# D-Robotics/hobot_stereonet

Measured on AMD Instinct MI355X. Metric: stereo pairs/s at 1280x720 D=192 (ms/frame alongside), higher is better.
Workload: dtype f16 (refinement-tower MFMA operands fp16 — 3x3 weights rounded per kernel so that every kernel's tap sum survives —, LeakyReLU applied after the fp16 rounding; low-resolution branch on 22-bit hi/lo split fp16 operands, 3 fp16 MFMAs per product in every 32-channel layer — profiles/r04_lowres_ablation

## Files before the change

hobot_stereonet_amd/csrc/sn_stream_block.hpp:

```cpp
#pragma once

#ifdef SN_STREAM_TIMING
#define SN_STAMP(k)                                                                                   \
  do {                                                                                                \
    if (blockIdx.x == 17 && q >= 8 && q < 24) {                                                       \
      const unsigned long long t_ = __builtin_readcyclecounter();                                     \
      if (lane == 0) reinterpret_cast<unsigned long long*>(dump + 64)[(wave * 16 + q - 8) * 8 + (k)] = t_; \
    }                                                                                                 \
  } while (0)
#define SN_STAMP_WG(k)                                                                                          \
  do {                                                                                                          \
    if (threadIdx.x == 0) {                                                                                     \
      unsigned long long* d_ = reinterpret_cast<unsigned long long*>(dump + 64) + 1152 + 4 * blockIdx.x + (k);  \
      d_[0] = __builtin_readcyclecounter();                                                                     \
      d_[2] = wall_clock64();                                                                                   \
    }                                                                                                           \
  } while (0)
#else
#define SN_STAMP(k) do { } while (0)
#define SN_STAMP_WG(k) do { } while (0)
#endif

namespace sn {

// ... 9 lines not shown
  static constexpr int LAG = HEAD_ ? 3 : 2;
  static constexpr int PROWS = 2 * R + 2;
  static constexpr int PRING_BYTES = HEAD_ ? PROWS * 9 * TW * 4 : 0;
  static constexpr int WIN_BYTES = HEAD_ ? NWR_ * 2 * 64 * 4 : 0;
  static constexpr int XW = TW + 2 * DIL;
  static constexpr int CSEG = TW / 32;
  static constexpr int SPW = R * CSEG / NWR;
  static constexpr int XROW = 4 * XW, TROW = 4 * TW;
  static constexpr int XGROUP = R * XROW;
  static constexpr int NINST = (XGROUP + 63) / 64;
  static constexpr int KW = (NINST + NWR - 1) / NWR;
  static constexpr int XGP = NINST * 64;
  static constexpr int TGP = R * TROW;
  static constexpr int XRING = NXS * XGP;
  static constexpr int TRING = NTS * TGP + 64;
  static constexpr int LDS_BYTES = (XRING + TRING) * 16 + 2 * 2 * 16 * 4 + PRING_BYTES + WIN_BYTES;
  static constexpr int ROWS_ABOVE = (R + HS) * DIL, ROWS_BELOW = (R + 2 + HS) * DIL - 1;
  static_assert(!HEAD_ || (DIL_ == 1 && R_ == 4 && TW_ == 64 && NWR_ == 4), "the tail form is written for the dilation-1 strip shape");
  static_assert(SPW == 1 || SPW == 2, "segments per wave");
  static_assert(CSEG % SPW == 0, "a wave's segments lie in one row");
  static_assert(PF == 2, "prefetch distance the counted waits are written for");
  static_assert(R == 4 || R == 2, "rows per step");
  static_assert(LDS_BYTES <= 160 * 1024, "one workgroup per CU");
};

struct StreamSched {
  int nstrips;
  int hsub;
  int total_rows;
  int rows_per_wg;
};

template <int R, int HS = 0>
struct StreamIter {
  int f, f_end, hsub;
  int sp, v0, v1, n, j, live;
  __device__ __forceinline__ void next_unit() {
    if (f >= f_end) { live = 0; return; }
    sp = f / hsub;
    v0 = f - sp * hsub;
    int L = hsub - v0;
    if (L > f_end - f) L = f_end - f;
    v1 = v0 + L;
    n = (L + 2 + 2 * HS + R - 1) / R;
    j = 0;
    f += L;
    live = 1;
  }
  __device__ __forceinline__ void step(int q, int lag, int f0, int f1, int hsub_) {
    if (q < lag) { live = 0; return; }
    if (q == lag) { f = f0; f_end = f1; hsub = hsub_; next_unit(); return; }
    if (live && ++j > n) next_unit();
  }
};

__device__ __forceinline__ unsigned lrelu_pack2(float a, float b) { return act_pack2_f16(a, b, (_Float16)kSlope); }

template <int HI>
__device__ __forceinline__ float res_add(unsigned r, float acc) {
  float d;
  if (HI) asm("v_fma_mix_f32 %0, %1, 1.0, %2 op_sel:[1,0,0] op_sel_hi:[1,0,0]" : "=v"(d) : "v"(r), "v"(acc));
  else asm("v_fma_mix_f32 %0, %1, 1.0, %2 op_sel_hi:[1,0,0]" : "=v"(d) : "v"(r), "v"(acc));
  return d;
}

__device__ __forceinline__ unsigned lds_addr(const void* p) {
  return (unsigned)(size_t)(const __attribute__((address_space(3))) void*)p;
}

// ... 33 lines not shown
  }
  __builtin_amdgcn_sched_group_barrier(0x008, AHEAD, 0);
}

__device__ __forceinline__ void glds16(unsigned lds_dst, unsigned voff, const void* base) {
  unsigned keep;
  asm volatile(
      "s_mov_b32 %0, m0\n\t"
      "s_mov_b32 m0, %1\n\t"
      "s_nop 0\n\t"
      "global_load_lds_dwordx4 %2, %3\n\t"
      "s_mov_b32 m0, %0"
      : "=&s"(keep)
      : "s"(lds_dst), "v"(voff), "s"(base)
      : "memory");
}

__device__ __forceinline__ void glds4(unsigned lds_dst, unsigned voff, const void* base) {
  unsigned keep;
  asm volatile(
      "s_mov_b32 %0, m0\n\t"
      "s_mov_b32 m0, %1\n\t"
      "s_nop 0\n\t"
      "global_load_lds_dword %2, %3\n\t"
      "s_mov_b32 m0, %0"
      : "=&s"(keep)
      : "s"(lds_dst), "v"(voff), "s"(base)
      : "memory");
}

// ... 3 lines not shown
                                                                const uint4* __restrict__ wfrag2, const float* __restrict__ bias2,
                                                                RefGeom g, StreamSched sc, uint4* __restrict__ dump, HeadArgs ha) {
  using T = StreamTile<DIL, TW, R, NXS, NWR, HEAD>;
  constexpr int HS = T::HS;
  extern __shared__ __attribute__((aligned(16))) uint4 lds[];
  uint4* const xring = lds;
  uint4* const tring = lds + T::XRING;
  float* const s_bias = reinterpret_cast<float*>(tring + T::TRING);
  float* const pring = s_bias + 64;
  float* const s_win = pring + T::PRING_BYTES / 4;
  const int tid = threadIdx.x, lane = tid & 63;
  const int wave = __builtin_amdgcn_readfirstlane(tid >> 6);
  const int j = lane & 31, gh = lane >> 5;
  const int role = wave / NWR, rw = wave % NWR;

  const int f0 = (int)blockIdx.x * sc.rows_per_wg;
  int f1 = f0 + sc.rows_per_wg;
  if (f1 > sc.total_rows) f1 = sc.total_rows;
  if (f0 >= f1) return;
  SN_STAMP_WG(0);
  int nss = T::LAG;
  for (int f = f0; f < f1;) {
    const int v0 = f % sc.hsub;
    int L = sc.hsub - v0;
    if (L > f1 - f) L = f1 - f;
    nss += (L + 2 + 2 * HS + R - 1) / R + 1;
    f += L;
  }
  auto decode_sp = [&](int sp, int& img, int& py, int& x0) {
    const int t = sp / sc.nstrips;
    x0 = (sp - t * sc.nstrips) * T::OW + T::X0OFF;
    img = t / DIL;
    py = t - img * DIL;
  };
  const unsigned plane_b = (unsigned)g.Hs * (unsigned)g.Ws * 16u;

  half8 wf[18];
  {
    const uint4* wsrc = role ? wfrag2 : wfrag1;
#pragma unroll
    for (int i = 0; i < 18; ++i) {
      const uint4 a = wsrc[i * 64 + lane];
      wf[i] = *reinterpret_cast<const half8*>(&a);
    }
    if (tid < 64) {
      const int c = tid >> 5, g2 = (tid >> 4) & 1, r = tid & 15;
      s_bias[tid] = (c ? bias2 : bias1)[(r & 3) + 8 * (r >> 2) + 4 * g2];
    }
#pragma unroll
// ... 12 lines not shown
    const int lane_w = cseg0 * 32 + j;
    constexpr int KWMAX = T::KW;
    const int kw = (T::NINST - rw + NWR - 1) / NWR;
    unsigned dma_voff[KWMAX];
#pragma unroll
    for (int k = 0; k < KWMAX; ++k) {
      const int i = rw + NWR * k;
      int s = i * 64 + lane;
      s = s < T::XGROUP ? s : T::XGROUP - 1;
      const int r = s / T::XROW;
      const int rem = s - r * T::XROW;
      const int blk = rem / T::XW;
      const int c = rem - blk * T::XW;
      dma_voff[k] = (unsigned)blk * plane_b + ((unsigned)(r * DIL) * (unsigned)g.Ws + (unsigned)c) * 16u;
    }
    long last_base = 0;
    auto dma_issue = [&](const StreamIter<R, HS>& it, int grp) {
      if (it.live) {
        int img, py, x0;
        decode_sp(it.sp, img, py, x0);
        const int row = (it.v0 - HS - R + R * it.j) * DIL + py;
        last_base = (((long)img * 4 * g.Hs + (row + kRefPad)) * (long)g.Ws + (x0 - 2 * DIL + kRefPad)) * 16;
      }
      const char* src = reinterpret_cast<const char*>(xin) + last_base;
      const unsigned dst = lds_addr(xring + grp * T::XGP);
#pragma unroll
      for (int k = 0; k < KWMAX; ++k)
        if (k < kw) glds16(dst + (unsigned)(rw + NWR * k) * 1024u, dma_voff[k], src);
    };
    auto wait_group = [&](auto extra) {
      constexpr int E = decltype(extra)::value;
      if (kw == KWMAX) wait_vmcnt<KWMAX + E>();
      else wait_vmcnt<KWMAX - 1 + E>();
    };
    StreamIter<R, HS> dm, c1, fin, fin2;
    dm.live = c1.live = fin.live = fin2.live = 0;
    int fin_img = 0, fin_x0 = 0, fin2_img = 0, fin2_x0 = 0;
    auto win_first_col = [&](int xs) {
      float sx = ((float)xs + 0.5f) * ha.ups.rs - 0.5f;
      sx = sx < 0.f ? 0.f : sx;
      return (int)sx;
    };
    int p4 = 0;
    unsigned long long moved = 0ull;
    unsigned bad = 0u;
    dm.step(0, 0, f0, f1, sc.hsub);
    dma_issue(dm, 0);
    dm.step(1, 0, f0, f1, sc.hsub);
    dma_issue(dm, 1);
    wait_group(std::integral_constant<int, 0>{});
    block_barrier();

    int c1_py = 0, c1_x0 = 0;
    int qx = 0, qt = 0;
    for (int q = 0; q < nss; ++q) {
      dm.step(q + 2, 0, f0, f1, sc.hsub);
      c1.step(q, 0, f0, f1, sc.hsub);
      const int do1 = c1.live && c1.j >= 1;
      const int gx0 = qx, gx1 = qx >= 1 ? qx - 1 : qx - 1 + NXS;
      const int gxp = qx + 2 >= NXS ? qx + 2 - NXS : qx + 2;
      SN_STAMP(0);
      if constexpr (HEAD) {
        fin.step(q, 3, f0, f1, sc.hsub);
        if (fin.live && fin.j >= 1) {
          if (fin.j == 1) {
            int py;
            decode_sp(fin.sp, fin_img, py, fin_x0);
          }
          const int o = fin.v0 - 4 + R * (fin.j - 1) + rowW;
          if (o >= fin.v0 && o < fin.v1 && o < ha.H) {
            const int pb = p4 + 8 >= T::PROWS ? p4 + 8 - T::PROWS : p4 + 8;
            float acc = ha.bias;
#pragma unroll
            for (int ky = 0; ky < 3; ++ky) {
              int pr = pb + rowW - 2 + ky;
              pr = pr < 0 ? pr + T::PROWS : (pr >= T::PROWS ? pr - T::PROWS : pr);
              const float* prow = pring + pr * (9 * TW) + lane - 1;
#pragma unroll
              for (int kx = 0; kx < 3; ++kx) acc += prow[(ky * 3 + kx) * TW + kx];
            }
            const int X = fin_x0 + lane;
            float sy = ((float)o + 0.5f) * ha.ups.rs - 0.5f;
            float sx = ((float)X + 0.5f) * ha.ups.rs - 0.5f;
            sy = sy < 0.f ? 0.f : sy;
            sx = sx < 0.f ? 0.f : sx;
            const int y0 = (int)sy, x0 = (int)sx;
            const int x1 = x0 < ha.wl - 1 ? x0 + 1 : x0;
            const float ly = sy - (float)y0, lx = sx - (float)x0;
            const float hy = 1.0f - ly, hx = 1.0f - lx;
            const int cb = win_first_col(fin_x0);
            const float* w0 = s_win + rw * 128;
            const float v = hy * (hx * w0[x0 - cb] + lx * w0[x1 - cb]) + ly * (hx * w0[64 + x0 - cb] + lx * w0[64 + x1 - cb]);
            const float up = v * ha.ups.mul;
            float mv;
            unsigned nf;
            const float d = head_value(up, ha.dmax, acc, mv, nf);
            if (lane >= 1 && lane <= T::OW && X < ha.W) {
              moved += stat_fixed(mv);
              bad += nf;
              head_store(ha.out_disp, ha.out_raw, ((size_t)fin_img * ha.H + o) * ha.W + X, d, ha.inv_q);
            }
          }
        }
      }
      if constexpr (HEAD) {
        fin2.step(q, 2, f0, f1, sc.hsub);
        if (fin2.live && fin2.j >= 1) {
          if (fin2.j == 1) {
            int py;
            decode_sp(fin2.sp, fin2_img, py, fin2_x0);
          }
          const int o = fin2.v0 - 4 + R * (fin2.j - 1) + rowW;
          if (o >= fin2.v0 && o < fin2.v1 && o < ha.H) {
            float sy = ((float)o + 0.5f) * ha.ups.rs - 0.5f;
            sy = sy < 0.f ? 0.f : sy;
            const int y0 = (int)sy;
            const int y1 = y0 < ha.hl - 1 ? y0 + 1 : y0;
            int c = win_first_col(fin2_x0) + lane;
            c = c < ha.wl - 1 ? c : ha.wl - 1;
            const float* lowp = ha.disp_low + (size_t)fin2_img * ha.hl * ha.wl;
            const unsigned dst = lds_addr(s_win + rw * 128);
            asm volatile("s_waitcnt lgkmcnt(0)" ::: "memory");
            glds4(dst, (unsigned)c * 4u, lowp + (size_t)y0 * ha.wl);
            glds4(dst + 256u, (unsigned)c * 4u, lowp + (size_t)y1 * ha.wl);
          }
        }
      }
      dma_issue(dm, gxp);
      SN_STAMP(1);
      if (do1) {
        if (c1.j == 1) {
          int img;
          decode_sp(c1.sp, img, c1_py, c1_x0);
        }
        const uint4* xp[3];
#pragma unroll
        for (int ky = 0; ky < 3; ++ky) {
          const int rr = rowW - 2 + ky;
          xp[ky] = xring + (rr < 0 ? gx1 : gx0) * T::XGP + (rr & (R - 1)) * T::XROW + lane_x;
        }
        const f32x16 bv = *reinterpret_cast<const f32x16*>(s_bias + gh * 16);
        f32x16 acc[T::SPW];
        stream_conv36<DIL, T::XW, T::SPW>(xp, wf, bv, acc);
        SN_STAMP(2);
        const int trow = (c1.v0 - HS - 1 + R * (c1.j - 1) + rowW) * DIL + c1_py;
        const bool row_ok = trow >= 0 && trow < g.H;
        const int tc0 = c1_x0 - DIL;
        const bool interior = row_ok && tc0 >= 0 && tc0 + TW <= g.W;
        uint4* tw = tring + qt * T::TGP + rowW * T::TROW + lane_w;
        auto write_t = [&](auto is_interior) {
#pragma unroll
          for (int s = 0; s < T::SPW; ++s) {
            bool inside = true;
            if (!decltype(is_interior)::value) {
              const int c = tc0 + (cseg0 + s) * 32 + j;
              inside = row_ok && c >= 0 && c < g.W;
            }
            unsigned pk[4][2];
#pragma unroll
            for (int qd = 0; qd < 4; ++qd)
// ... 14 lines not shown
      wait_group(std::integral_constant<int, 0>{});
      asm volatile("s_waitcnt lgkmcnt(0)" ::: "memory");
      SN_STAMP(4);
      block_barrier();
      qx = qx + 1 == NXS ? 0 : qx + 1;
      qt = qt + 1 == T::NTS ? 0 : qt + 1;
      p4 = p4 + R >= T::PROWS ? p4 + R - T::PROWS : p4 + R;
    }
    if constexpr (HEAD) refine_stat_commit_fixed(ha.stat, moved, bad);
    SN_STAMP_WG(1);
  } else {
    const int lane_t = gh * T::TW + cseg0 * 32 + j;
    const int lane_y = 2 * DIL + cseg0 * 32 + j;
    block_barrier();

    StreamIter<R, HS> c2, ep;
    c2.live = ep.live = 0;
    half8 ah[2], al[2];
    uint2 rres[T::SPW][4];
    int p4 = 0;
    if constexpr (HEAD) {
#pragma unroll
      for (int kk = 0; kk < 2; ++kk)
#pragma unroll
        for (int e = 0; e < 8; ++e) {
          const float wv = j < 9 ? ha.w[(16 * kk + 8 * gh + e) * 9 + j] : 0.f;
          const _Float16 hi = (_Float16)wv;
          ah[kk][e] = hi;
          al[kk][e] = (_Float16)((wv - (float)hi) * kSplitScale);
        }
#pragma unroll
      for (int s = 0; s < T::SPW; ++s)
#pragma unroll
        for (int qd = 0; qd < 4; ++qd) rres[s][qd] = uint2{0u, 0u};
    }
    int ep_img = 0, ep_py = 0, ep_x0 = 0;
    const unsigned lane_o = (unsigned)(cseg0 * 32 + j) * 16u + (unsigned)(2 * gh) * plane_b;
    f32x16 acc[T::SPW];
#pragma unroll
    for (int s = 0; s < T::SPW; ++s)
#pragma unroll
      for (int r = 0; r < 16; ++r) acc[s][r] = 0.f;
    int qx = 0, qt = 0;
    for (int q = 0; q < nss; ++q) {
      c2.step(q, 1, f0, f1, sc.hsub);
      ep.step(q, 2, f0, f1, sc.hsub);
      const int do2 = c2.live && c2.j >= 1;
      const int doe = ep.live && ep.j >= 1;
      const int gx2 = qx >= 2 ? qx - 2 : qx - 2 + NXS, gx3 = qx >= 3 ? qx - 3 : qx - 3 + NXS;
      const int gt1 = qt >= 1 ? qt - 1 : qt - 1 + T::NTS, gt2 = qt >= 2 ? qt - 2 : qt - 2 + T::NTS;
      SN_STAMP(0);
      if (doe) {
        if (ep.j == 1) decode_sp(ep.sp, ep_img, ep_py, ep_x0);
        const int sub = ep.v0 - HS - 2 + R * (ep.j - 1) + rowW;
        const int row = sub * DIL + ep_py;
        if constexpr (HEAD) {
          const bool row_ok = row >= 0 && row < g.H;
          const bool interior = row_ok && ep_x0 >= 0 && ep_x0 + TW <= g.W;
          int prow = p4 + 2 + rowW;
          prow = prow >= T::PROWS ? prow - T::PROWS : prow;
#pragma unroll
          for (int s = 0; s < T::SPW; ++s) {
            const int col = ep_x0 + (cseg0 + s) * 32 + j;
            const bool ok = row_ok && col >= 0 && col < g.W;
            unsigned pk[4][2];
#pragma unroll
            for (int qd = 0; qd < 4; ++qd) {
              const half4 rv = *reinterpret_cast<const half4*>(&rres[s][qd]);
              const uint2 rw2 = *reinterpret_cast<const uint2*>(&rv);
// ... 16 lines not shown
#pragma unroll
            for (int kk = 0; kk < 2; ++kk) {
              const auto r0 = __builtin_amdgcn_permlane32_swap(pk[2 * kk][0], pk[2 * kk + 1][0], false, false);
              const auto r1 = __builtin_amdgcn_permlane32_swap(pk[2 * kk][1], pk[2 * kk + 1][1], false, false);
              const uint4 sl = uint4{r0[0], r1[0], r0[1], r1[1]};
              const half8 xh = *reinterpret_cast<const half8*>(&sl);
              a0 = __builtin_amdgcn_mfma_f32_32x32x16_f16(ah[kk], xh, a0, 0, 0, 0);
              a1 = __builtin_amdgcn_mfma_f32_32x32x16_f16(al[kk], xh, a1, 0, 0, 0);
            }
            float* dst = pring + prow * (9 * TW) + (cseg0 + s) * 32 + j;
#pragma unroll
            for (int r = 0; r < 4; ++r) dst[(4 * gh + r) * TW] = a0[r] + a1[r] * kSplitInv;
            if (gh == 0) dst[8 * TW] = a0[4] + a1[4] * kSplitInv;
          }
        } else
        if (sub >= ep.v0 && sub < ep.v1 && row < g.H) {
          const int rr = rowW - 2;
          const uint4* xrow = xring + (rr < 0 ? gx3 : gx2) * T::XGP + (rr & (R - 1)) * T::XROW + lane_y;
          const unsigned ob = (((unsigned)ep_img * 4u * (unsigned)g.Hs + (unsigned)(row + kRefPad)) * (unsigned)g.Ws +
                               (unsigned)(ep_x0 + kRefPad)) * 16u;
#pragma unroll
          for (int s = 0; s < T::SPW; ++s) {
            unsigned pk[4][2];
#pragma unroll
            for (int qd = 0; qd < 4; ++qd) {
              const half4 rv = *reinterpret_cast<const half4*>(reinterpret_cast<const char*>(xrow + qd * T::XW + s * 32) + gh * 8);
              const uint2 rw2 = *reinterpret_cast<const uint2*>(&rv);
              pk[qd][0] = lrelu_pack2(res_add<0>(rw2.x, acc[s][4 * qd]), res_add<1>(rw2.x, acc[s][4 * qd + 1]));
              pk[qd][1] = lrelu_pack2(res_add<0>(rw2.y, acc[s][4 * qd + 2]), res_add<1>(rw2.y, acc[s][4 * qd + 3]));
            }
            uint4 sl[2];
#pragma unroll
            for (int k = 0; k < 2; ++k) {
              const auto r0 = __builtin_amdgcn_permlane32_swap(pk[k][0], pk[k + 2][0], false, false);
              const auto r1 = __builtin_amdgcn_permlane32_swap(pk[k][1], pk[k + 2][1], false, false);
// ... 47 lines not shown
```

hobot_stereonet_amd/csrc/sn_stream_block_x3.hpp:

```cpp
#pragma once

namespace sn {

template <int DIL_, int TW_ = 64, int R_ = 2, int NXS_ = 5, int NWR_ = 2>
struct StreamTileX3 {
  static constexpr int DIL = DIL_, TW = TW_, R = R_, NXS = NXS_, NTS = 3, PF = NXS_ - 3;
  static constexpr int NWR = NWR_;
  static constexpr int OW = TW - 2 * DIL;
  static constexpr int XW = TW + 2 * DIL;
  static constexpr int CSEG = TW / 32;
  static constexpr int SPW = R * CSEG / NWR;
  static constexpr int XROW = 4 * XW, TROW = 4 * TW;
  static constexpr int XGROUP = R * XROW;
  static constexpr int NINST = (XGROUP + 63) / 64;
  static constexpr int KW = (2 * NINST + NWR - 1) / NWR;
  static constexpr int XGP = NINST * 64;
  static constexpr int TGP = R * TROW;
  static constexpr int XRING = NXS * XGP;
  static constexpr int TRING = NTS * TGP + 64;
  static constexpr int LDS_BYTES = 2 * (XRING + TRING) * 16 + 2 * 2 * 16 * 4;
  static constexpr int ROWS_ABOVE = R * DIL, ROWS_BELOW = (R + 2) * DIL - 1;
  static_assert(SPW == 1 || SPW == 2, "segments per wave");
  static_assert(CSEG % SPW == 0, "a wave's segments lie in one row");
  static_assert(PF == 2, "prefetch distance the counted waits are written for");
  static_assert(R == 2 || R == 4, "rows per step");
  static_assert(LDS_BYTES <= 160 * 1024, "one workgroup per CU");
  static_assert(ROWS_ABOVE <= 2 * kRefPad, "a strip's first group stays inside the zero rows above an image (border + the plane before)");
};

__device__ __forceinline__ float x3_acc(float a0, float a1) { return a0 + a1 * kSplitInv; }

template <int DIL, int COLW, int SPW, int PART, bool DB = true>
__device__ __forceinline__ void stream_conv108(const uint4* const (&rp)[3], const half8 (&wh)[18], const half8 (&wl)[18],
                                               const f32x16& bv, f32x16 (&a0)[SPW], f32x16 (&a1)[SPW]) {
  constexpr int NB = 3 * SPW;
// ... 48 lines not shown

template <int DIL, int TW, int R, int NXS, int NWR>
__global__ __launch_bounds__(128 * NWR, NWR / 2) __attribute__((amdgpu_waves_per_eu(NWR / 2, NWR / 2))) void k_ref_block_stream_x3(
    const uint4* __restrict__ xin, uint4* __restrict__ yout, size_t lo_bytes, const uint4* __restrict__ wfrag1,
    const float* __restrict__ bias1, const uint4* __restrict__ wfrag2, const float* __restrict__ bias2, RefGeom g, StreamSched sc) {
  using T = StreamTileX3<DIL, TW, R, NXS, NWR>;
  extern __shared__ __attribute__((aligned(16))) uint4 lds[];
  uint4* const xring = lds;
  uint4* const tring = lds + 2 * T::XRING;
  float* const s_bias = reinterpret_cast<float*>(tring + 2 * T::TRING);
  const int tid = threadIdx.x, lane = tid & 63;
  const int wave = __builtin_amdgcn_readfirstlane(tid >> 6);
  const int j = lane & 31, gh = lane >> 5;
  const int role = wave / NWR, rw = wave % NWR;

  const int f0 = (int)blockIdx.x * sc.rows_per_wg;
  int f1 = f0 + sc.rows_per_wg;
  if (f1 > sc.total_rows) f1 = sc.total_rows;
  if (f0 >= f1) return;
  int nss = 2;
  for (int f = f0; f < f1;) {
    const int v0 = f % sc.hsub;
    int L = sc.hsub - v0;
    if (L > f1 - f) L = f1 - f;
    nss += (L + 2 + R - 1) / R + 1;
    f += L;
  }
  auto decode_sp = [&](int sp, int& img, int& py, int& x0) {
    const int t = sp / sc.nstrips;
    x0 = (sp - t * sc.nstrips) * T::OW;
    img = t / DIL;
    py = t - img * DIL;
  };
  const unsigned plane_b = (unsigned)g.Hs * (unsigned)g.Ws * 16u;

  half8 wfh[18], wfl[18];
  {
    const uint4* wsrc = role ? wfrag2 : wfrag1;
#pragma unroll
    for (int i = 0; i < 18; ++i) {
      const uint4 a = wsrc[i * 64 + lane], b = wsrc[(18 + i) * 64 + lane];
      wfh[i] = *reinterpret_cast<const half8*>(&a);
      wfl[i] = *reinterpret_cast<const half8*>(&b);
    }
    if (tid < 64) {
      const int c = tid >> 5, g2 = (tid >> 4) & 1, r = tid & 15;
      s_bias[tid] = (c ? bias2 : bias1)[(r & 3) + 8 * (r >> 2) + 4 * g2];
    }
// ... 15 lines not shown
    constexpr int KWMAX = T::KW;
    const int kw = (2 * T::NINST - rw + NWR - 1) / NWR;
    unsigned dma_voff[KWMAX];
#pragma unroll
    for (int k = 0; k < KWMAX; ++k) {
      int i = rw + NWR * k;
      i = i < T::NINST ? i : i - T::NINST;
      int s = i * 64 + lane;
      s = s < T::XGROUP ? s : T::XGROUP - 1;
      const int r = s / T::XROW;
      const int rem = s - r * T::XROW;
      const int blk = rem / T::XW;
      const int c = rem - blk * T::XW;
      dma_voff[k] = (unsigned)blk * plane_b + ((unsigned)(r * DIL) * (unsigned)g.Ws + (unsigned)c) * 16u;
    }
    long last_base = 0;
    auto dma_issue = [&](const StreamIter<R, 0>& it, int grp) {
      if (it.live) {
        int img, py, x0;
        decode_sp(it.sp, img, py, x0);
        const int row = (it.v0 - R + R * it.j) * DIL + py;
        last_base = (((long)img * 4 * g.Hs + (row + kRefPad)) * (long)g.Ws + (x0 - 2 * DIL + kRefPad)) * 16;
      }
      const char* src = reinterpret_cast<const char*>(xin) + last_base;
      const unsigned dst = lds_addr(xring + grp * T::XGP);
#pragma unroll
      for (int k = 0; k < KWMAX; ++k)
        if (k < kw) {
          const int i = rw + NWR * k;
          const bool lo = i >= T::NINST;
          const int ii = lo ? i - T::NINST : i;
          glds16(dst + (lo ? (unsigned)T::XRING * 16u : 0u) + (unsigned)ii * 1024u, dma_voff[k], src + (lo ? lo_bytes : (size_t)0));
        }
    };
    auto wait_group = [&]() {
      if (kw == KWMAX) wait_vmcnt<KWMAX>();
      else wait_vmcnt<KWMAX - 1>();
    };
    StreamIter<R, 0> dm, c1;
    dm.live = c1.live = 0;
    dm.step(0, 0, f0, f1, sc.hsub);
    dma_issue(dm, 0);
    dm.step(1, 0, f0, f1, sc.hsub);
    dma_issue(dm, 1);
    wait_group();
    block_barrier();

    int c1_py = 0, c1_x0 = 0;
    int qx = 0, qt = 0;
    for (int q = 0; q < nss; ++q) {
      dm.step(q + 2, 0, f0, f1, sc.hsub);
      c1.step(q, 0, f0, f1, sc.hsub);
      const int do1 = c1.live && c1.j >= 1;
      const int gx0 = qx, gx1 = qx >= 1 ? qx - 1 : qx - 1 + NXS;
      const int gxp = qx + 2 >= NXS ? qx + 2 - NXS : qx + 2;
      dma_issue(dm, gxp);
      if (do1) {
        if (c1.j == 1) {
          int img;
          decode_sp(c1.sp, img, c1_py, c1_x0);
        }
        const uint4* xp[3];
#pragma unroll
        for (int ky = 0; ky < 3; ++ky) {
          const int rr = rowW - 2 + ky;
          xp[ky] = xring + (rr < 0 ? gx1 : gx0) * T::XGP + (rr & (R - 1)) * T::XROW + lane_x;
        }
        const f32x16 bv = *reinterpret_cast<const f32x16*>(s_bias + gh * 16);
        f32x16 a0[T::SPW], a1[T::SPW];
        stream_conv108<DIL, T::XW, T::SPW, T::XRING, (NWR <= 2)>(xp, wfh, wfl, bv, a0, a1);
        const int trow = (c1.v0 - 1 + R * (c1.j - 1) + rowW) * DIL + c1_py;
        const bool row_ok = trow >= 0 && trow < g.H;
        const int tc0 = c1_x0 - DIL;
        uint4* tw = tring + qt * T::TGP + rowW * T::TROW + lane_w;
#pragma unroll
        for (int s = 0; s < T::SPW; ++s) {
          const int c = tc0 + (cseg0 + s) * 32 + j;
          const bool inside = row_ok && c >= 0 && c < g.W;
#pragma unroll
          for (int qd = 0; qd < 4; ++qd) {
            half4 hh, hl;
#pragma unroll
            for (int e = 0; e < 4; ++e) {
              float v = x3_acc(a0[s][4 * qd + e], a1[s][4 * qd + e]);
              v = lrelu_fast(v);
              const _Float16 hi = (_Float16)v;
// ... 9 lines not shown
            *reinterpret_cast<half4*>(dst + (size_t)T::TRING * 16) = hl;
          }
        }
      }
      wait_group();
      asm volatile("s_waitcnt lgkmcnt(0)" ::: "memory");
      block_barrier();
      qx = qx + 1 == NXS ? 0 : qx + 1;
      qt = qt + 1 == T::NTS ? 0 : qt + 1;
    }
  } else {
    const int lane_t = gh * T::TW + cseg0 * 32 + j;
    const int lane_y = 2 * DIL + cseg0 * 32 + j;
    block_barrier();

    StreamIter<R, 0> c2, ep;
    c2.live = ep.live = 0;
    int ep_img = 0, ep_py = 0, ep_x0 = 0;
    const unsigned lane_o = (unsigned)(cseg0 * 32 + j) * 16u + (unsigned)(2 * gh) * plane_b;
    f32x16 a0[T::SPW], a1[T::SPW];
    uint2 rrh[T::SPW][4], rrl[T::SPW][4];
#pragma unroll
    for (int s = 0; s < T::SPW; ++s) {
#pragma unroll
      for (int r = 0; r < 16; ++r) {
        a0[s][r] = 0.f;
        a1[s][r] = 0.f;
      }
#pragma unroll
      for (int qd = 0; qd < 4; ++qd) {
        rrh[s][qd] = uint2{0u, 0u};
        rrl[s][qd] = uint2{0u, 0u};
      }
    }
    int qx = 0, qt = 0;
    for (int q = 0; q < nss; ++q) {
      c2.step(q, 1, f0, f1, sc.hsub);
      ep.step(q, 2, f0, f1, sc.hsub);
      const int do2 = c2.live && c2.j >= 1;
      const int doe = ep.live && ep.j >= 1;
      const int gx1 = qx >= 1 ? qx - 1 : qx - 1 + NXS, gx2 = qx >= 2 ? qx - 2 : qx - 2 + NXS;
      const int gt1 = qt >= 1 ? qt - 1 : qt - 1 + T::NTS, gt2 = qt >= 2 ? qt - 2 : qt - 2 + T::NTS;
      if (doe) {
        if (ep.j == 1) decode_sp(ep.sp, ep_img, ep_py, ep_x0);
        const int sub = ep.v0 - 2 + R * (ep.j - 1) + rowW;
        const int row = sub * DIL + ep_py;
        if (sub >= ep.v0 && sub < ep.v1 && row < g.H) {
          const unsigned ob = (((unsigned)ep_img * 4u * (unsigned)g.Hs + (unsigned)(row + kRefPad)) * (unsigned)g.Ws +
                               (unsigned)(ep_x0 + kRefPad)) * 16u;
#pragma unroll
          for (int s = 0; s < T::SPW; ++s) {
            unsigned ph[4][2], pl[4][2];
#pragma unroll
            for (int qd = 0; qd < 4; ++qd) {
              const half4 vh = *reinterpret_cast<const half4*>(&rrh[s][qd]);
              const half4 vl = *reinterpret_cast<const half4*>(&rrl[s][qd]);
              half4 hh, hl;
#pragma unroll
              for (int e = 0; e < 4; ++e) {
                float v = x3_acc(a0[s][4 * qd + e], a1[s][4 * qd + e]);
                v += (float)vh[e] + (float)vl[e] * kSplitInv;
                v = lrelu_fast(v);
                const _Float16 hi = (_Float16)v;
                hh[e] = hi;
// ... 64 lines not shown
```

Before: 3009.

## Precompute per-unit strip descriptors into an LDS ring table for streaming kernels

Moves per-unit strip decoding (integer divides for strip/image/phase, DMA base, output base, window column) out of every pipeline cursor and into a small LDS ring table. Wave 0 fills the table at start and one wave refills half of it as the DMA cursor advances. Cursors read the entries with readfirstlane into scalars, and the DMA base advances by a fixed pitch instead of being recomputed each step. This removes repeated scalar division and address arithmetic from the streaming loop. In exchange it adds LDS footprint, a table-refill dependency between waves, and more complex cursor logic.

```diff
diff --git a/hobot_stereonet_amd/csrc/sn_stream_block.hpp b/hobot_stereonet_amd/csrc/sn_stream_block.hpp
--- a/hobot_stereonet_amd/csrc/sn_stream_block.hpp
+++ b/hobot_stereonet_amd/csrc/sn_stream_block.hpp
@@ -1,4 +1,6 @@
 #pragma once
+
+#include "sn_stream_units.hpp"
 
 #ifdef SN_STREAM_TIMING
 #define SN_STAMP(k)                                                                                   \
@@ -47,7 +49,7 @@
   static constexpr int TGP = R * TROW;
   static constexpr int XRING = NXS * XGP;
   static constexpr int TRING = NTS * TGP + 64;
-  static constexpr int LDS_BYTES = (XRING + TRING) * 16 + 2 * 2 * 16 * 4 + PRING_BYTES + WIN_BYTES;
+  static constexpr int LDS_BYTES = (XRING + TRING) * 16 + 2 * 2 * 16 * 4 + PRING_BYTES + WIN_BYTES + kStreamUnitBytes;
   static constexpr int ROWS_ABOVE = (R + HS) * DIL, ROWS_BELOW = (R + 2 + HS) * DIL - 1;
   static_assert(!HEAD_ || (DIL_ == 1 && R_ == 4 && TW_ == 64 && NWR_ == 4), "the tail form is written for the dilation-1 strip shape");
   static_assert(SPW == 1 || SPW == 2, "segments per wave");
@@ -57,35 +59,67 @@
   static_assert(LDS_BYTES <= 160 * 1024, "one workgroup per CU");
 };
 
-struct StreamSched {
-  int nstrips;
-  int hsub;
-  int total_rows;
-  int rows_per_wg;
+struct StreamCursor {
+  int u, j, n, live;
+  __device__ __forceinline__ bool step(int q, int lag, int nu) {
+    if (q < lag) { live = 0; return false; }
+    if (q == lag) { u = 0; j = 0; live = 1; return true; }
+    if (!live || ++j <= n) return false;
+    j = 0;
+    if (++u < nu) return true;
+    live = 0;
+    return false;
+  }
 };
 
-template <int R, int HS = 0>
-struct StreamIter {
-  int f, f_end, hsub;
-  int sp, v0, v1, n, j, live;
-  __device__ __forceinline__ void next_unit() {
-    if (f >= f_end) { live = 0; return; }
-    sp = f / hsub;
-    v0 = f - sp * hsub;
-    int L = hsub - v0;
-    if (L > f_end - f) L = f_end - f;
-    v1 = v0 + L;
-    n = (L + 2 + 2 * HS + R - 1) / R;
-    j = 0;
-    f += L;
-    live = 1;
-  }
-  __device__ __forceinline__ void step(int q, int lag, int f0, int f1, int hsub_) {
-    if (q < lag) { live = 0; return; }
-    if (q == lag) { f = f0; f_end = f1; hsub = hsub_; next_unit(); return; }
-    if (live && ++j > n) next_unit();
-  }
-};
+__device__ __forceinline__ int4 stream_unit_words(const int4* tab, int u, int w4) {
+  const int4 v = tab[(u & (kStreamUnitRing - 1)) * 4 + w4];
+  return int4{__builtin_amdgcn_readfirstlane(v.x), __builtin_amdgcn_readfirstlane(v.y), __builtin_amdgcn_readfirstlane(v.z),
+              __builtin_amdgcn_readfirstlane(v.w)};
+}
+
+template <int DIL, int R, int HS, int OW, int X0OFF>
+__device__ __forceinline__ void stream_units_write(int4* tab, const StreamSched& sc, const StreamShare& sh, const StreamUnitGeom& ug,
+                                                   int u0, int count, int lane) {
+  if (lane < count) {
+    const StreamUnit t = stream_unit<DIL, R, HS, OW, X0OFF>(sc, sh, ug, u0 + lane);
+    int4* d = tab + ((u0 + lane) & (kStreamUnitRing - 1)) * 4;
+    d[0] = int4{t.sp, t.v0, t.v1, t.n};
+    d[1] = int4{t.img, t.py, t.x0, t.slot0};
+    d[2] = int4{t.dma_lo, t.dma_hi, (int)t.ybase, t.wcol};
+  }
+}
+template <int DIL, int R, int HS, int OW, int X0OFF>
+__device__ __forceinline__ void stream_units_init(int4* tab, const StreamSched& sc, const StreamShare& sh, const StreamUnitGeom& ug,
+                                                  int lane) {
+  stream_units_write<DIL, R, HS, OW, X0OFF>(tab, sc, sh, ug, 0, kStreamUnitRing, lane);
+  if (lane == 0) {
+    int4* d = tab + kStreamUnitRing * 4;
+    d[0] = int4{sc.nstrips, sc.hsub, sh.f0, sh.f1};
+    d[1] = int4{sh.sp0, sh.n0, sh.nfull, 0};
+    d[2] = int4{ug.Hs, ug.Ws, ug.pad, __float_as_int(ug.rs)};
+  }
+}
+template <int DIL, int R, int HS, int OW, int X0OFF>
+__device__ __forceinline__ void stream_units_refill(int4* tab, int u, int lane) {
+  if (u >= kStreamUnitRing - kStreamUnitHalf / 2 && (u & (kStreamUnitHalf - 1)) == kStreamUnitHalf / 2) {
+    const int4* h = tab + kStreamUnitRing * 4;
+    const int4 a = h[0], b = h[1], c = h[2];
+    StreamSched sc;
+    sc.nstrips = a.x;
+    sc.hsub = a.y;
+    sc.total_rows = sc.rows_per_wg = 0;
+    StreamShare sh;
+    sh.f0 = a.z;
+    sh.f1 = a.w;
+    sh.sp0 = b.x;
+    sh.n0 = b.y;
+    sh.nfull = b.z;
+    sh.nu = sh.nslots = 0;
+    const StreamUnitGeom ug{c.x, c.y, c.z, __int_as_float(c.w)};
+    stream_units_write<DIL, R, HS, OW, X0OFF>(tab, sc, sh, ug, u + kStreamUnitHalf / 2, kStreamUnitHalf, lane);
+  }
+}
 
 __device__ __forceinline__ unsigned lrelu_pack2(float a, float b) { return act_pack2_f16(a, b, (_Float16)kSlope); }
 
@@ -149,6 +183,12 @@
       : "=&s"(keep)
       : "s"(lds_dst), "v"(voff), "s"(base)
       : "memory");
+}
+
+__device__ __forceinline__ const void* uniform_ptr(const void* p) {
+  const unsigned long long v = (unsigned long long)p;
+  const unsigned lo = __builtin_amdgcn_readfirstlane((unsigned)v), hi = __builtin_amdgcn_readfirstlane((unsigned)(v >> 32));
+  return reinterpret_cast<const void*>(((unsigned long long)hi << 32) | lo);
 }
 
 __device__ __forceinline__ void glds4(unsigned lds_dst, unsigned voff, const void* base) {
@@ -182,25 +222,14 @@
   const int j = lane & 31, gh = lane >> 5;
   const int role = wave / NWR, rw = wave % NWR;
 
-  const int f0 = (int)blockIdx.x * sc.rows_per_wg;
-  int f1 = f0 + sc.rows_per_wg;
-  if (f1 > sc.total_rows) f1 = sc.total_rows;
-  if (f0 >= f1) return;
+  int4* const s_units = reinterpret_cast<int4*>(s_win + T::WIN_BYTES / 4);
+  const StreamShare sh = stream_share<R, HS>(sc, (int)blockIdx.x);
+  if (sh.nu == 0) return;
   SN_STAMP_WG(0);
-  int nss = T::LAG;
-  for (int f = f0; f < f1;) {
-    const int v0 = f % sc.hsub;
-    int L = sc.hsub - v0;
-    if (L > f1 - f) L = f1 - f;
-    nss += (L + 2 + 2 * HS + R - 1) / R + 1;
-    f += L;
-  }
-  auto decode_sp = [&](int sp, int& img, int& py, int& x0) {
-    const int t = sp / sc.nstrips;
-    x0 = (sp - t * sc.nstrips) * T::OW + T::X0OFF;
-    img = t / DIL;
-    py = t - img * DIL;
-  };
+  const int nu = sh.nu;
+  const int nss = T::LAG + sh.nslots;
+  const StreamUnitGeom ug{g.Hs, g.Ws, kRefPad, HEAD ? ha.ups.rs : 0.f};
+  if (wave == 0) stream_units_init<DIL, R, HS, T::OW, T::X0OFF>(s_units, sc, sh, ug, lane);
   const unsigned plane_b = (unsigned)g.Hs * (unsigned)g.Ws * 16u;
 
   half8 wf[18];
@@ -243,15 +272,29 @@
       const int c = rem - blk * T::XW;
       dma_voff[k] = (unsigned)blk * plane_b + ((unsigned)(r * DIL) * (unsigned)g.Ws + (unsigned)c) * 16u;
     }
-    long last_base = 0;
-    auto dma_issue = [&](const StreamIter<R, HS>& it, int grp) {
-      if (it.live) {
-        int img, py, x0;
-        decode_sp(it.sp, img, py, x0);
-        const int row = (it.v0 - HS - R + R * it.j) * DIL + py;
-        last_base = (((long)img * 4 * g.Hs + (row + kRefPad)) * (long)g.Ws + (x0 - 2 * DIL + kRefPad)) * 16;
-      }
-      const char* src = reinterpret_cast<const char*>(xin) + last_base;
+    long dm_base = 0;
+    const long dm_pitch = (long)(R * DIL) * (long)g.Ws * 16;
+    StreamCursor dm;
+    {
+      const StreamUnit t0 = stream_unit<DIL, R, HS, T::OW, T::X0OFF>(sc, sh, ug, 0);
+      dm.u = 0;
+      dm.j = 0;
+      dm.n = t0.n;
+      dm.live = 1;
+      dm_base = (long)(((unsigned long long)(unsigned)t0.dma_hi << 32) | (unsigned long long)(unsigned)t0.dma_lo);
+    }
+    auto dm_step = [&](int q) {
+      if (dm.step(q, 0, nu)) {
+        const int4 a = stream_unit_words(s_units, dm.u, 0), c = stream_unit_words(s_units, dm.u, 2);
+        dm.n = a.w;
+        dm_base = (long)(((unsigned long long)(unsigned)c.y << 32) | (unsigned long long)(unsigned)c.x);
+        if (rw == 0) stream_units_refill<DIL, R, HS, T::OW, T::X0OFF>(s_units, dm.u, lane);
+      } else if (dm.live) {
+        dm_base += dm_pitch;
+      }
+    };
+    auto dma_issue = [&](int grp) {
+      const char* src = reinterpret_cast<const char*>(xin) + dm_base;
       const unsigned dst = lds_addr(xring + grp * T::XGP);
 #pragma unroll
       for (int k = 0; k < KWMAX; ++k)
@@ -262,42 +305,37 @@
       if (kw == KWMAX) wait_vmcnt<KWMAX + E>();
       else wait_vmcnt<KWMAX - 1 + E>();
     };
-    StreamIter<R, HS> dm, c1, fin, fin2;
-    dm.live = c1.live = fin.live = fin2.live = 0;
-    int fin_img = 0, fin_x0 = 0, fin2_img = 0, fin2_x0 = 0;
-    auto win_first_col = [&](int xs) {
-      float sx = ((float)xs + 0.5f) * ha.ups.rs - 0.5f;
-      sx = sx < 0.f ? 0.f : sx;
-      return (int)sx;
-    };
+    StreamCursor c1, fin2;
+    c1.live = fin2.live = 0;
+    int fin2_v0 = 0, fin2_v1 = 0, fin2_img = 0, fin2_x0 = 0, fin2_cb = 0;
+    int fin_do = 0, fin_o = 0, fin_img = 0, fin_x0 = 0, fin_cb = 0;
     int p4 = 0;
     unsigned long long moved = 0ull;
     unsigned bad = 0u;
-    dm.step(0, 0, f0, f1, sc.hsub);
-    dma_issue(dm, 0);
-    dm.step(1, 0, f0, f1, sc.hsub);
-    dma_issue(dm, 1);
+    dma_issue(0);
+    dm_step(1);
+    dma_issue(1);
     wait_group(std::integral_constant<int, 0>{});
     block_barrier();
 
-    int c1_py = 0, c1_x0 = 0;
+    int c1_trow0 = 0, c1_x0 = 0;
     int qx = 0, qt = 0;
     for (int q = 0; q < nss; ++q) {
-      dm.step(q + 2, 0, f0, f1, sc.hsub);
-      c1.step(q, 0, f0, f1, sc.hsub);
+      dm_step(q + 2);
+      if (c1.step(q, 0, nu)) {
+        const int4 a = stream_unit_words(s_units, c1.u, 0), b = stream_unit_words(s_units, c1.u, 1);
+        c1.n = a.w;
+        c1_trow0 = (a.y - HS - 1) * DIL + b.y;
+        c1_x0 = b.z;
+      }
       const int do1 = c1.live && c1.j >= 1;
       const int gx0 = qx, gx1 = qx >= 1 ? qx - 1 : qx - 1 + NXS;
       const int gxp = qx + 2 >= NXS ? qx + 2 - NXS : qx + 2;
       SN_STAMP(0);
       if constexpr (HEAD) {
-        fin.step(q, 3, f0, f1, sc.hsub);
-        if (fin.live && fin.j >= 1) {
-          if (fin.j == 1) {
-            int py;
-            decode_sp(fin.sp, fin_img, py, fin_x0);
-          }
-          const int o = fin.v0 - 4 + R * (fin.j - 1) + rowW;
-          if (o >= fin.v0 && o < fin.v1 && o < ha.H) {
+        {
+          const int o = fin_o;
+          if (fin_do) {
             const int pb = p4 + 8 >= T::PROWS ? p4 + 8 - T::PROWS : p4 + 8;
             float acc = ha.bias;
 #pragma unroll
@@ -317,7 +355,7 @@
             const int x1 = x0 < ha.wl - 1 ? x0 + 1 : x0;
             const float ly = sy - (float)y0, lx = sx - (float)x0;
             const float hy = 1.0f - ly, hx = 1.0f - lx;
-            const int cb = win_first_col(fin_x0);
+            const int cb = fin_cb;
             const float* w0 = s_win + rw * 128;
             const float v = hy * (hx * w0[x0 - cb] + lx * w0[x1 - cb]) + ly * (hx * w0[64 + x0 - cb] + lx * w0[64 + x1 - cb]);
             const float up = v * ha.ups.mul;
@@ -333,35 +371,41 @@
         }
       }
       if constexpr (HEAD) {
-        fin2.step(q, 2, f0, f1, sc.hsub);
+        if (fin2.step(q, 2, nu)) {
+          const int4 a = stream_unit_words(s_units, fin2.u, 0), b = stream_unit_words(s_units, fin2.u, 1), c = stream_unit_words(s_units, fin2.u, 2);
+          fin2.n = a.w;
+          fin2_v0 = a.y;
+          fin2_v1 = a.z;
+          fin2_img = b.x;
+          fin2_x0 = b.z;
+          fin2_cb = c.w;
+        }
+        fin_do = 0;
+        fin_img = fin2_img;
+        fin_x0 = fin2_x0;
+        fin_cb = fin2_cb;
         if (fin2.live && fin2.j >= 1) {
-          if (fin2.j == 1) {
-            int py;
-            decode_sp(fin2.sp, fin2_img, py, fin2_x0);
-          }
-          const int o = fin2.v0 - 4 + R * (fin2.j - 1) + rowW;
-          if (o >= fin2.v0 && o < fin2.v1 && o < ha.H) {
+          const int o = fin2_v0 - 4 + R * (fin2.j - 1) + rowW;
+          if (o >= fin2_v0 && o < fin2_v1 && o < ha.H) {
+            fin_do = 1;
+            fin_o = o;
             float sy = ((float)o + 0.5f) * ha.ups.rs - 0.5f;
             sy = sy < 0.f ? 0.f : sy;
             const int y0 = (int)sy;
             const int y1 = y0 < ha.hl - 1 ? y0 + 1 : y0;
-            int c = win_first_col(fin2_x0) + lane;
+            int c = fin2_cb + lane;
             c = c < ha.wl - 1 ? c : ha.wl - 1;
             const float* lowp = ha.disp_low + (size_t)fin2_img * ha.hl * ha.wl;
             const unsigned dst = lds_addr(s_win + rw * 128);
             asm volatile("s_waitcnt lgkmcnt(0)" ::: "memory");
-            glds4(dst, (unsigned)c * 4u, lowp + (size_t)y0 * ha.wl);
-            glds4(dst + 256u, (unsigned)c * 4u, lowp + (size_t)y1 * ha.wl);
+            glds4(dst, (unsigned)c * 4u, uniform_ptr(lowp + (size_t)y0 * ha.wl));
+            glds4(dst + 256u, (unsigned)c * 4u, uniform_ptr(lowp + (size_t)y1 * ha.wl));
           }
         }
       }
-      dma_issue(dm, gxp);
+      dma_issue(gxp);
       SN_STAMP(1);
       if (do1) {
-        if (c1.j == 1) {
-          int img;
-          decode_sp(c1.sp, img, c1_py, c1_x0);
-        }
         const uint4* xp[3];
 #pragma unroll
         for (int ky = 0; ky < 3; ++ky) {
@@ -372,7 +416,7 @@
         f32x16 acc[T::SPW];
         stream_conv36<DIL, T::XW, T::SPW>(xp, wf, bv, acc);
         SN_STAMP(2);
-        const int trow = (c1.v0 - HS - 1 + R * (c1.j - 1) + rowW) * DIL + c1_py;
+        const int trow = c1_trow0 + (R * (c1.j - 1) + rowW) * DIL;
         const bool row_ok = trow >= 0 && trow < g.H;
         const int tc0 = c1_x0 - DIL;
         const bool interior = row_ok && tc0 >= 0 && tc0 + TW <= g.W;
@@ -417,7 +461,7 @@
     const int lane_y = 2 * DIL + cseg0 * 32 + j;
     block_barrier();
 
-    StreamIter<R, HS> c2, ep;
+    StreamCursor c2, ep;
     c2.live = ep.live = 0;
     half8 ah[2], al[2];
     uint2 rres[T::SPW][4];
@@ -437,7 +481,8 @@
 #pragma unroll
         for (int qd = 0; qd < 4; ++qd) rres[s][qd] = uint2{0u, 0u};
     }
-    int ep_img = 0, ep_py = 0, ep_x0 = 0;
+    int ep_v0 = 0, ep_v1 = 0, ep_py = 0, ep_x0 = 0;
+    unsigned ep_ybase = 0u;
     const unsigned lane_o = (unsigned)(cseg0 * 32 + j) * 16u + (unsigned)(2 * gh) * plane_b;
     f32x16 acc[T::SPW];
 #pragma unroll
@@ -446,16 +491,23 @@
       for (int r = 0; r < 16; ++r) acc[s][r] = 0.f;
     int qx = 0, qt = 0;
     for (int q = 0; q < nss; ++q) {
-      c2.step(q, 1, f0, f1, sc.hsub);
-      ep.step(q, 2, f0, f1, sc.hsub);
+      if (c2.step(q, 1, nu)) c2.n = stream_unit_words(s_units, c2.u, 0).w;
+      if (ep.step(q, 2, nu)) {
+        const int4 a = stream_unit_words(s_units, ep.u, 0), b = stream_unit_words(s_units, ep.u, 1), c = stream_unit_words(s_units, ep.u, 2);
+        ep.n = a.w;
+        ep_v0 = a.y;
+        ep_v1 = a.z;
+        ep_py = b.y;
+        ep_x0 = b.z;
+        ep_ybase = (unsigned)c.z;
+      }
       const int do2 = c2.live && c2.j >= 1;
       const int doe = ep.live && ep.j >= 1;
       const int gx2 = qx >= 2 ? qx - 2 : qx - 2 + NXS, gx3 = qx >= 3 ? qx - 3 : qx - 3 + NXS;
       const int gt1 = qt >= 1 ? qt - 1 : qt - 1 + T::NTS, gt2 = qt >= 2 ? qt - 2 : qt - 2 + T::NTS;
       SN_STAMP(0);
       if (doe) {
-        if (ep.j == 1) decode_sp(ep.sp, ep_img, ep_py, ep_x0);
-        const int sub = ep.v0 - HS - 2 + R * (ep.j - 1) + rowW;
+        const int sub = ep_v0 - HS - 2 + R * (ep.j - 1) + rowW;
         const int row = sub * DIL + ep_py;
         if constexpr (HEAD) {
           const bool row_ok = row >= 0 && row < g.H;
@@ -502,11 +554,10 @@
             if (gh == 0) dst[8 * TW] = a0[4] + a1[4] * kSplitInv;
           }
         } else
-        if (sub >= ep.v0 && sub < ep.v1 && row < g.H) {
+        if (sub >= ep_v0 && sub < ep_v1 && row < g.H) {
           const int rr = rowW - 2;
           const uint4* xrow = xring + (rr < 0 ? gx3 : gx2) * T::XGP + (rr & (R - 1)) * T::XROW + lane_y;
-          const unsigned ob = (((unsigned)ep_img * 4u * (unsigned)g.Hs + (unsigned)(row + kRefPad)) * (unsigned)g.Ws +
-                               (unsigned)(ep_x0 + kRefPad)) * 16u;
+          const unsigned ob = ep_ybase + (unsigned)(sub * DIL) * (unsigned)g.Ws * 16u;
 #pragma unroll
           for (int s = 0; s < T::SPW; ++s) {
             unsigned pk[4][2];
diff --git a/hobot_stereonet_amd/csrc/sn_stream_block_x3.hpp b/hobot_stereonet_amd/csrc/sn_stream_block_x3.hpp
--- a/hobot_stereonet_amd/csrc/sn_stream_block_x3.hpp
+++ b/hobot_stereonet_amd/csrc/sn_stream_block_x3.hpp
@@ -18,7 +18,7 @@
   static constexpr int TGP = R * TROW;
   static constexpr int XRING = NXS * XGP;
   static constexpr int TRING = NTS * TGP + 64;
-  static constexpr int LDS_BYTES = 2 * (XRING + TRING) * 16 + 2 * 2 * 16 * 4;
+  static constexpr int LDS_BYTES = 2 * (XRING + TRING) * 16 + 2 * 2 * 16 * 4 + kStreamUnitBytes;
   static constexpr int ROWS_ABOVE = R * DIL, ROWS_BELOW = (R + 2) * DIL - 1;
   static_assert(SPW == 1 || SPW == 2, "segments per wave");
   static_assert(CSEG % SPW == 0, "a wave's segments lie in one row");
@@ -97,24 +97,13 @@
   const int j = lane & 31, gh = lane >> 5;
   const int role = wave / NWR, rw = wave % NWR;
 
-  const int f0 = (int)blockIdx.x * sc.rows_per_wg;
-  int f1 = f0 + sc.rows_per_wg;
-  if (f1 > sc.total_rows) f1 = sc.total_rows;
-  if (f0 >= f1) return;
-  int nss = 2;
-  for (int f = f0; f < f1;) {
-    const int v0 = f % sc.hsub;
-    int L = sc.hsub - v0;
-    if (L > f1 - f) L = f1 - f;
-    nss += (L + 2 + R - 1) / R + 1;
-    f += L;
-  }
-  auto decode_sp = [&](int sp, int& img, int& py, int& x0) {
-    const int t = sp / sc.nstrips;
-    x0 = (sp - t * sc.nstrips) * T::OW;
-    img = t / DIL;
-    py = t - img * DIL;
-  };
+  int4* const s_units = reinterpret_cast<int4*>(s_bias + 64);
+  const StreamShare sh = stream_share<R, 0>(sc, (int)blockIdx.x);
+  if (sh.nu == 0) return;
+  const int nu = sh.nu;
+  const int nss = 2 + sh.nslots;
+  const StreamUnitGeom ug{g.Hs, g.Ws, kRefPad, 0.f};
+  if (wave == 0) stream_units_init<DIL, R, 0, T::OW, 0>(s_units, sc, sh, ug, lane);
   const unsigned plane_b = (unsigned)g.Hs * (unsigned)g.Ws * 16u;
 
   half8 wfh[18], wfl[18];
@@ -160,15 +149,29 @@
       const int c = rem - blk * T::XW;
       dma_voff[k] = (unsigned)blk * plane_b + ((unsigned)(r * DIL) * (unsigned)g.Ws + (unsigned)c) * 16u;
     }
-    long last_base = 0;
-    auto dma_issue = [&](const StreamIter<R, 0>& it, int grp) {
-      if (it.live) {
-        int img, py, x0;
-        decode_sp(it.sp, img, py, x0);
-        const int row = (it.v0 - R + R * it.j) * DIL + py;
-        last_base = (((long)img * 4 * g.Hs + (row + kRefPad)) * (long)g.Ws + (x0 - 2 * DIL + kRefPad)) * 16;
-      }
-      const char* src = reinterpret_cast<const char*>(xin) + last_base;
+    long dm_base = 0;
+    const long dm_pitch = (long)(R * DIL) * (long)g.Ws * 16;
+    StreamCursor dm;
+    {
+      const StreamUnit t0 = stream_unit<DIL, R, 0, T::OW, 0>(sc, sh, ug, 0);
+      dm.u = 0;
+      dm.j = 0;
+      dm.n = t0.n;
+      dm.live = 1;
+      dm_base = (long)(((unsigned long long)(unsigned)t0.dma_hi << 32) | (unsigned long long)(unsigned)t0.dma_lo);
+    }
+    auto dm_step = [&](int q) {
+      if (dm.step(q, 0, nu)) {
+        const int4 a = stream_unit_words(s_units, dm.u, 0), c = stream_unit_words(s_units, dm.u, 2);
+        dm.n = a.w;
+        dm_base = (long)(((unsigned long long)(unsigned)c.y << 32) | (unsigned long long)(unsigned)c.x);
+        if (rw == 0) stream_units_refill<DIL, R, 0, T::OW, 0>(s_units, dm.u, lane);
+      } else if (dm.live) {
+        dm_base += dm_pitch;
+      }
+    };
+    auto dma_issue = [&](int grp) {
+      const char* src = reinterpret_cast<const char*>(xin) + dm_base;
       const unsigned dst = lds_addr(xring + grp * T::XGP);
 #pragma unroll
       for (int k = 0; k < KWMAX; ++k)
@@ -183,29 +186,29 @@
       if (kw == KWMAX) wait_vmcnt<KWMAX>();
       else wait_vmcnt<KWMAX - 1>();
     };
-    StreamIter<R, 0> dm, c1;
-    dm.live = c1.live = 0;
-    dm.step(0, 0, f0, f1, sc.hsub);
-    dma_issue(dm, 0);
-    dm.step(1, 0, f0, f1, sc.hsub);
-    dma_issue(dm, 1);
+    StreamCursor c1;
+    c1.live = 0;
+    dma_issue(0);
+    dm_step(1);
+    dma_issue(1);
     wait_group();
     block_barrier();
 
-    int c1_py = 0, c1_x0 = 0;
+    int c1_trow0 = 0, c1_x0 = 0;
     int qx = 0, qt = 0;
     for (int q = 0; q < nss; ++q) {
-      dm.step(q + 2, 0, f0, f1, sc.hsub);
-      c1.step(q, 0, f0, f1, sc.hsub);
+      dm_step(q + 2);
+      if (c1.step(q, 0, nu)) {
+        const int4 a = stream_unit_words(s_units, c1.u, 0), b = stream_unit_words(s_units, c1.u, 1);
+        c1.n = a.w;
+        c1_trow0 = (a.y - 1) * DIL + b.y;
+        c1_x0 = b.z;
+      }
       const int do1 = c1.live && c1.j >= 1;
       const int gx0 = qx, gx1 = qx >= 1 ? qx - 1 : qx - 1 + NXS;
       const int gxp = qx + 2 >= NXS ? qx + 2 - NXS : qx + 2;
-      dma_issue(dm, gxp);
+      dma_issue(gxp);
       if (do1) {
-        if (c1.j == 1) {
-          int img;
-          decode_sp(c1.sp, img, c1_py, c1_x0);
-        }
         const uint4* xp[3];
 #pragma unroll
         for (int ky = 0; ky < 3; ++ky) {
@@ -215,7 +218,7 @@
         const f32x16 bv = *reinterpret_cast<const f32x16*>(s_bias + gh * 16);
         f32x16 a0[T::SPW], a1[T::SPW];
         stream_conv108<DIL, T::XW, T::SPW, T::XRING, (NWR <= 2)>(xp, wfh, wfl, bv, a0, a1);
-        const int trow = (c1.v0 - 1 + R * (c1.j - 1) + rowW) * DIL + c1_py;
+        const int trow = c1_trow0 + (R * (c1.j - 1) + rowW) * DIL;
         const bool row_ok = trow >= 0 && trow < g.H;
         const int tc0 = c1_x0 - DIL;
         uint4* tw = tring + qt * T::TGP + rowW * T::TROW + lane_w;
@@ -255,9 +258,10 @@
     const int lane_y = 2 * DIL + cseg0 * 32 + j;
     block_barrier();
 
-    StreamIter<R, 0> c2, ep;
+    StreamCursor c2, ep;
     c2.live = ep.live = 0;
-    int ep_img = 0, ep_py = 0, ep_x0 = 0;
+    int ep_v0 = 0, ep_v1 = 0, ep_py = 0, ep_x0 = 0;
+    unsigned ep_ybase = 0u;
     const unsigned lane_o = (unsigned)(cseg0 * 32 + j) * 16u + (unsigned)(2 * gh) * plane_b;
     f32x16 a0[T::SPW], a1[T::SPW];
     uint2 rrh[T::SPW][4], rrl[T::SPW][4];
@@ -276,19 +280,25 @@
     }
     int qx = 0, qt = 0;
     for (int q = 0; q < nss; ++q) {
-      c2.step(q, 1, f0, f1, sc.hsub);
-      ep.step(q, 2, f0, f1, sc.hsub);
+      if (c2.step(q, 1, nu)) c2.n = stream_unit_words(s_units, c2.u, 0).w;
+      if (ep.step(q, 2, nu)) {
+        const int4 a = stream_unit_words(s_units, ep.u, 0), b = stream_unit_words(s_units, ep.u, 1), c = stream_unit_words(s_units, ep.u, 2);
+        ep.n = a.w;
+        ep_v0 = a.y;
+        ep_v1 = a.z;
+        ep_py = b.y;
+        ep_x0 = b.z;
+        ep_ybase = (unsigned)c.z;
+      }
       const int do2 = c2.live && c2.j >= 1;
       const int doe = ep.live && ep.j >= 1;
       const int gx1 = qx >= 1 ? qx - 1 : qx - 1 + NXS, gx2 = qx >= 2 ? qx - 2 : qx - 2 + NXS;
       const int gt1 = qt >= 1 ? qt - 1 : qt - 1 + T::NTS, gt2 = qt >= 2 ? qt - 2 : qt - 2 + T::NTS;
       if (doe) {
-        if (ep.j == 1) decode_sp(ep.sp, ep_img, ep_py, ep_x0);
-        const int sub = ep.v0 - 2 + R * (ep.j - 1) + rowW;
+        const int sub = ep_v0 - 2 + R * (ep.j - 1) + rowW;
         const int row = sub * DIL + ep_py;
-        if (sub >= ep.v0 && sub < ep.v1 && row < g.H) {
-          const unsigned ob = (((unsigned)ep_img * 4u * (unsigned)g.Hs + (unsigned)(row + kRefPad)) * (unsigned)g.Ws +
-                               (unsigned)(ep_x0 + kRefPad)) * 16u;
+        if (sub >= ep_v0 && sub < ep_v1 && row < g.H) {
+          const unsigned ob = ep_ybase + (unsigned)(sub * DIL) * (unsigned)g.Ws * 16u;
 #pragma unroll
           for (int s = 0; s < T::SPW; ++s) {
             unsigned ph[4][2], pl[4][2];
diff --git a/hobot_stereonet_amd/csrc/sn_stream_units.hpp b/hobot_stereonet_amd/csrc/sn_stream_units.hpp
--- /dev/null
+++ b/hobot_stereonet_amd/csrc/sn_stream_units.hpp
@@ -0,0 +1,99 @@
+#pragma once
+
+#if defined(__HIPCC__) || defined(__CUDACC__)
+#define SN_HD __host__ __device__ __forceinline__
+#else
+#define SN_HD inline
+#endif
+
+namespace sn {
+
+struct StreamSched {
+  int nstrips;
+  int hsub;
+  int total_rows;
+  int rows_per_wg;
+};
+
+struct StreamUnit {
+  int sp, v0, v1, n;
+  int img, py, x0, slot0;
+  int dma_lo, dma_hi;
+  unsigned ybase;
+  int wcol;
+  int pad[4];
+};
+static_assert(sizeof(StreamUnit) == 64, "four LDS slots per unit");
+
+constexpr int kStreamUnitRing = 16;
+constexpr int kStreamUnitHalf = kStreamUnitRing / 2;
+constexpr int kStreamUnitBytes = (kStreamUnitRing + 1) * (int)sizeof(StreamUnit);
+
+struct StreamUnitGeom {
+  int Hs, Ws, pad;
+  float rs;
+};
+
+struct StreamShare {
+  int f0, f1;
+  int sp0, nu;
+  int n0, nfull;
+  int nslots;
+};
+
+template <int R, int HS>
+SN_HD int stream_unit_steps(int L) { return (L + 2 + 2 * HS + R - 1) / R; }
+
+template <int R, int HS>
+SN_HD StreamShare stream_share(const StreamSched& sc, int wg) {
+  StreamShare s;
+  s.f0 = wg * sc.rows_per_wg;
+  s.f1 = s.f0 + sc.rows_per_wg;
+  if (s.f1 > sc.total_rows) s.f1 = sc.total_rows;
+  s.sp0 = 0;
+  s.nu = 0;
+  s.n0 = s.nfull = s.nslots = 0;
+  if (s.f0 >= s.f1) return s;
+  s.sp0 = s.f0 / sc.hsub;
+  s.nu = (s.f1 + sc.hsub - 1) / sc.hsub - s.sp0;
+  const int v0 = s.f0 - s.sp0 * sc.hsub;
+  int L0 = sc.hsub - v0;
+  if (L0 > s.f1 - s.f0) L0 = s.f1 - s.f0;
+  s.n0 = stream_unit_steps<R, HS>(L0);
+  s.nfull = stream_unit_steps<R, HS>(sc.hsub);
+  s.nslots = s.n0 + 1;
+  if (s.nu >= 2) {
+    const int Ll = s.f1 - (s.sp0 + s.nu - 1) * sc.hsub;
+    s.nslots += (s.nu - 2) * (s.nfull + 1) + stream_unit_steps<R, HS>(Ll) + 1;
+  }
+  return s;
+}
+
+template <int DIL, int R, int HS, int OW, int X0OFF>
+SN_HD StreamUnit stream_unit(const StreamSched& sc, const StreamShare& s, const StreamUnitGeom& g, int u) {
+  StreamUnit t;
+  t.sp = s.sp0 + u;
+  t.v0 = u == 0 ? s.f0 - s.sp0 * sc.hsub : 0;
+  int v1 = s.f1 - t.sp * sc.hsub;
+  t.v1 = v1 < sc.hsub ? v1 : sc.hsub;
+  t.n = stream_unit_steps<R, HS>(t.v1 - t.v0);
+  t.slot0 = u == 0 ? 0 : s.n0 + 1 + (u - 1) * (s.nfull + 1);
+  const int q = t.sp / sc.nstrips;
+  t.x0 = (t.sp - q * sc.nstrips) * OW + X0OFF;
+  t.img = q / DIL;
+  t.py = q - t.img * DIL;
+  const int row = (t.v0 - HS - R) * DIL + t.py;
+  const long long b = (((long long)t.img * 4 * g.Hs + (row + g.pad)) * (long long)g.Ws + (t.x0 - 2 * DIL + g.pad)) * 16;
+  t.dma_lo = (int)(unsigned)((unsigned long long)b & 0xffffffffull);
+  t.dma_hi = (int)(unsigned)((unsigned long long)b >> 32);
+  t.ybase = (((unsigned)t.img * 4u * (unsigned)g.Hs + (unsigned)(t.py + g.pad)) * (unsigned)g.Ws + (unsigned)(t.x0 + g.pad)) * 16u;
+  {
+    float sx = ((float)t.x0 + 0.5f) * g.rs - 0.5f;
+    sx = sx < 0.f ? 0.f : sx;
+    t.wcol = (int)sx;
+  }
+  t.pad[0] = t.pad[1] = t.pad[2] = t.pad[3] = 0;
+  return t;
+}
+
+}
```

Measured after the change: 3033, median of 6. About the same (+0.8%).
